# wvu-navLab/corenav-GP

Measured on AMD Instinct MI355X. Metric: GP-fits/s, higher is better.
Workload: dtype f64; 1 GPU; BASELINE configs[1]: batch of independent fixed-theta GP fits, N=2048 d=6 M=599 kernel=SE-ARD f64; streams=0, pipeline_depth=1, N=2048, d=6, M=599, inputs=resident in HBM, ranks=1

## Files before the change

### corenav_gp_amd/csrc/cgp_kernels_fused.hpp

```cpp
#pragma once
#include "cgp_kernels.hpp"

namespace cgp {

#ifndef CGP_SKIP_DEAD_WAVE
#define CGP_SKIP_DEAD_WAVE 1
#endif
constexpr bool kSkipDeadWave = CGP_SKIP_DEAD_WAVE != 0;

template <typename T>
__device__ __forceinline__ void stage_first_chunk(const T *gR, size_t ldR, const T *gC, size_t ldC, T *smem, int tid) {
  constexpr int CH = KT * LDST;
  if constexpr (sizeof(T) == 8) {
    typedef __attribute__((address_space(3))) void lds_void;
    typedef const __attribute__((address_space(1))) void gbl_void;
    const int lane = tid & 63;
    const int wave = __builtin_amdgcn_readfirstlane(tid >> 6);
#pragma unroll
    for (int i = 0; i < KT / 4; ++i) {
      const int col = wave * (KT / 4) + i;
      __builtin_amdgcn_global_load_lds((gbl_void *)(gR + (size_t)col * ldR + lane * 2), (lds_void *)(smem + col * LDST), 16, 0, 0);
      __builtin_amdgcn_global_load_lds((gbl_void *)(gC + (size_t)col * ldC + lane * 2), (lds_void *)(smem + CH + col * LDST), 16, 0, 0);
    }
  } else {
// ... 731 lines not shown
  const bf8 c01[2] = {__builtin_bit_cast(bf8, a01[RB0]), __builtin_bit_cast(bf8, a01[RB1])};
  static_for<0, RB1 + 1>([&](auto cc) {
    constexpr int CB = decltype(cc)::value;
    const bf8 a = __builtin_bit_cast(bf8, a01[CB]);
    if constexpr (CB <= RB0) acc[CB][0] = __builtin_amdgcn_mfma_f32_16x16x32_bf16(a, c10[0], acc[CB][0], 0, 0, 0);
    acc[CB][1] = __builtin_amdgcn_mfma_f32_16x16x32_bf16(a, c10[1], acc[CB][1], 0, 0, 0);
  });
  static_for<0, RB1 + 1>([&](auto cc) {
    constexpr int CB = decltype(cc)::value;
    const bf8 a = __builtin_bit_cast(bf8, a01[CB]);
    if constexpr (CB <= RB0) acc[CB][0] = __builtin_amdgcn_mfma_f32_16x16x32_bf16(a, c01[0], acc[CB][0], 0, 0, 0);
    acc[CB][1] = __builtin_amdgcn_mfma_f32_16x16x32_bf16(a, c01[1], acc[CB][1], 0, 0, 0);
  });
}
template <int D, int W, int S>
__device__ __forceinline__ void bx6_tri_iter(Prec<float>::acc_t (&acc)[NCB][2], BxTriStage<D> &st, int c, int nchunk, float *smem, const unsigned (&e)[2], bool hi) {
  st.template load<S>(c + D);
  lds_barrier();
  bx6_tri_compute<W, (S & 1) * 6 * BX_PLANE>(acc, e, hi);
  if (c + 1 < nchunk) st.template store<(S + 1) % D>(smem + ((S + 1) & 1) * BXT_FLOATS);
}
template <int D, int W>
__device__ __forceinline__ void bx6_tri_wave(Prec<float>::acc_t (&acc)[NCB][2], BxTriStage<D> &st, int nchunk, float *smem, int tid) {
  const int lane = tid & 63, l15 = lane & 15, lq = lane >> 4;
  const unsigned base = (unsigned)(size_t)smem;
  const unsigned e[2] = {base + 2 * bx_pos(l15, lq & 1), base + 2 * (bx_pos(DB + l15, lq & 1) - DB * BXS)};
  st.template store<0>(smem);
  for (int c0 = 0; c0 < nchunk; c0 += D) {
    bx6_tri_iter<D, W, 0>(acc, st, c0, nchunk, smem, e, lq >> 1);
    bx6_tri_iter<D, W, 1>(acc, st, c0 + 1, nchunk, smem, e, lq >> 1);
    if (D > 2) bx6_tri_iter<D, W, 2 % D>(acc, st, c0 + 2, nchunk, smem, e, lq >> 1);
    if (D > 2) bx6_tri_iter<D, W, 3 % D>(acc, st, c0 + 3, nchunk, smem, e, lq >> 1);
  }
}
template <int D>
__device__ __forceinline__ void bx6_syrk_tri_loop(Prec<float>::acc_t (&acc)[NCB][2], BxTriStage<D> &st, int nchunk, float *smem, int tid) {
  if (nchunk <= 0) return;
  const int wave = __builtin_amdgcn_readfirstlane(tid >> 6);
  switch (wave) {
    case 0: bx6_tri_wave<D, 0>(acc, st, nchunk, smem, tid); break;
    case 1: bx6_tri_wave<D, 1>(acc, st, nchunk, smem, tid); break;
    case 2: bx6_tri_wave<D, 2>(acc, st, nchunk, smem, tid); break;
    default: bx6_tri_wave<D, 3>(acc, st, nchunk, smem, tid); break;
  }
}

__device__ __forceinline__ double exp_gen(double x, const ExpC &e) { return exp_nonpos(x, e); }
__device__ __forceinline__ float exp_gen(float x, const ExpC &) { return __expf(fmaxf(x, -104.f)); }

constexpr int GK = 12;
template <bool DBL> constexpr int bx_z_offset() { return DBL ? 2 * BX_FLOATS : BX_FLOATS + 2 * GK * TS + 3 * TS; }
static_assert(2 * GK * TS + 3 * TS <= BX_FLOATS, "Gram inputs fit the second plane buffer");

template <typename T, bool BROWN, bool FAST, bool TRI = false, int NR = 2, bool DIFF1 = false, int MAT = 0>
__device__ __forceinline__ void gram_apply_tile(const FitArgs &p, typename Prec<T>::acc_t (&acc)[NCB][NR],
                                                const T *__restrict__ xrT, const T *__restrict__ xcT,
                                                const T *__restrict__ xraw, const T *__restrict__ craw,
                                                const T *__restrict__ yc, bool extra, int rowbase, int colbase, T amp,
                                                T amp_b, T diag_add, int lane, int wave, T inv_ell = T(0)) {
  using P = Prec<T>;
  using acc_t = typename P::acc_t;
  const int N = p.N, M = p.M, l15 = lane & 15, lq = lane >> 4;
  ExpC ec;
  ec.load();
  static_assert(NR == 2 || (NR == 1 && !TRI), "row blocks per wave");
  const int rbj[2] = {TRI ? wave : 0, TRI ? NCB - 1 - wave : 0};
  const int rl[2] = {TRI ? rbj[0] * DB + l15 : (NR == 2 ? wave * 32 + 2 * l15 : wave * DB + l15),
                     TRI ? rbj[1] * DB + l15 : wave * 32 + 2 * l15 + 1};
  T fb[NR][GK / 4];
#pragma unroll
  for (int j = 0; j < NR; ++j)
#pragma unroll
    for (int s = 0; s < GK / 4; ++s) fb[j][s] = xrT[(4 * s + lq) * TS + rl[j]];
  static_assert(!DIFF1 || (!BROWN && sizeof(T) == 4), "the difference form is for the fp32 SE kernels");
  static_assert(MAT == 0 || (!BROWN && !DIFF1 && sizeof(T) == 8), "the Matern kernels are fp64 cases of the inner-product form");
  T xrw[2] = {T(0), T(0)};
  if (BROWN || DIFF1) {
    xrw[0] = xraw[rl[0]];
    if (NR == 2) xrw[1] = xraw[rl[1]];
  }
#pragma unroll
  for (int cb = 0; cb < NCB; ++cb) {
    if (TRI && cb > rbj[0] && cb > rbj[1]) continue;
    T fa[GK / 4];
#pragma unroll
    for (int s = 0; s < GK / 4; ++s) fa[s] = xcT[(4 * s + lq) * TS + cb * DB + l15];
#pragma unroll
    for (int j = 0; j < NR; ++j) {
      if (TRI && cb > rbj[j]) continue;
      acc_t e = acc_t{0, 0, 0, 0};
      if constexpr (!DIFF1) {
#pragma unroll
        for (int s = 0; s < GK / 4; ++s) e = P::mfma(fa[s], fb[j][s], e);
      }
      const int grow = rowbase + rl[j];
#pragma unroll
      for (int r = 0; r < 4; ++r) {
        const int cl = cb * DB + P::drow(lane, r);
        const int gcol = colbase + cl;
        T g;
        if constexpr (DIFF1) {
          const T df = (xrw[j] - craw[cl]) * inv_ell;
          g = amp * exp_gen(T(-0.5) * df * df, ec);
        } else if constexpr (MAT != 0) {
          const bool same = !FAST && !extra && grow == gcol;
          double unused;
          g = amp * T(matern_radial<MAT == 2, false>(same ? 0.0 : -2.0 * (double)e[r], unused, [&](double x) { return exp_nonpos(x, ec); }));
        } else if (!BROWN) {
          g = CGP_DBG_ON(p, 128) ? e[r] : exp_gen(e[r], ec);
        } else {
          const T x = xrw[j], xp = craw[cl];
          const bool same = !FAST && !extra && grow == gcol;
          T ee = e[r] > T(0) ? T(0) : e[r];
          if constexpr (sizeof(T) == 4) {
            const T df = (x - xp) * inv_ell;
            ee = T(-0.5) * df * df;
          }
          ee = same ? T(0) : ee;
          const int sx = (x > T(0)) - (x < T(0)), sp = (xp > T(0)) - (xp < T(0));
          const T ax = x < T(0) ? -x : x, ap = xp < T(0) ? -xp : xp;
          const T kb = (sx == sp) ? amp_b * (ax < ap ? ax : ap) : T(0);
          g = amp * exp_gen(ee, ec) * kb;
        }
        if (!FAST) {
          const bool colok = gcol < N;
          if (!extra) {
            const bool dg = grow == gcol;
            g = dg ? g + diag_add : g;
            g = (grow < N && colok) ? g : (dg ? T(1) : T(0));
          } else {
            if (p.xid) g = (grow == gcol) ? T(1) : T(0);
            g = (grow == M) ? yc[cl] : g;
            g = (!colok || grow > M) ? T(0) : g;
          }
        }
        acc[cb][j][r] = -g;
      }
    }
    __builtin_amdgcn_sched_barrier(0);
  }
}

__global__ void k_prep(FitArgs p, int batch, double *prep, int zero_info, int *wready) {
  const int b = blockIdx.x * blockDim.x + threadIdx.x;
  if (b >= batch) return;
  if (zero_info) p.info[b] = 0;
  if (wready) wready[b] = 0;
  const double *th = p.theta + (size_t)b * MAX_THETA;
  double *o = prep + (size_t)b * PREP_N;
  const int kid = p.kernel_id, d = p.d;
  for (int q = 0; q < MAXD; ++q) {
    double s = 0.0;
    if (q < d) s = k_is_ard(kid) ? 1.0 / th[1 + q] : 1.0 / th[1];
    o[q] = s;
  }
  const bool brown = kid == K_RBF_BROWNIAN;
  o[8] = (brown || k_is_matern(kid)) ? 0.0 : log(th[0]);
  o[9] = th[0];
  o[10] = brown ? th[2] : 0.0;
  const int nth = k_ntheta(kid, d);
  o[11] = th[nth - 1] + 1e-8 + (p.jitter ? p.jitter[b] : 0.0);
  for (int q = 12; q < PREP_N; ++q) o[q] = 0.0;
}

template <typename T> struct GramPre {
  T v[MAXD];
  T yv;
};

template <typename T>
__device__ __forceinline__ void gram_prefetch(const FitArgs &p, int b, int k, int rt, int tid, GramPre<T> &g, int row0 = -1) {
  const int d = p.d, N = p.N, M = p.M;
  const bool extra = rt >= p.NT;
  const T *__restrict__ Xb = reinterpret_cast<const T *>(p.X) + (size_t)b * d * N;
  const T *__restrict__ Xsb = reinterpret_cast<const T *>(p.Xs) + (size_t)b * d * M;
  const T *__restrict__ yb = reinterpret_cast<const T *>(p.y) + (size_t)b * N;
  const bool isrow = tid < TS;
  const int r = tid & 127;
  const T *src = Xb;
  int idx, len = N;
  if (isrow) {
    if (!extra) idx = (row0 >= 0 ? row0 : rt * TS) + r;
    else { src = Xsb; idx = (row0 >= 0 ? row0 : (rt - p.NT) * TS) + r; len = M; }
  } else idx = k * TS + r;
  const bool ok = idx < len;
#pragma unroll
  for (int q = 0; q < MAXD; ++q) g.v[q] = (q < d && ok) ? src[(size_t)q * len + idx] : T(0);
  g.yv = (!isrow && ok) ? yb[idx] : T(0);
}

template <typename T, bool TRI = false, int NR = 2, bool MAT = false>
__device__ __forceinline__ void gram_apply(const FitArgs &p, typename Prec<T>::acc_t (&acc)[NCB][NR], T *__restrict__ smem,
                                           int b, int k, int rt, int tid, const GramPre<T> &g, PhaseClock *pc = nullptr,
                                           int slot = 0, int row0 = -1, bool live = true) {
  const double *__restrict__ pr = p.prep + (size_t)b * PREP_N;
  const int kid = p.kernel_id, N = p.N, M = p.M;
  const bool extra = rt >= p.NT;
  const bool brown = kid == K_RBF_BROWNIAN;
  const int lane = tid & 63;
  const int wave = __builtin_amdgcn_readfirstlane(tid >> 6);
  T *xrT = smem;
  T *xcT = smem + GK * TS;
  T *xraw = smem + 2 * GK * TS;
  T *craw = xraw + TS;
  T *yc = craw + TS;
  {
    const bool isrow = tid < TS;
    const int r = tid & 127;
    T *dst = isrow ? xrT : xcT;
    T nrm = 0;
#pragma unroll
    for (int q = 0; q < MAXD; ++q) {
      const T v = g.v[q] * T(pr[q]);
      nrm = __builtin_fma(v, v, nrm);
      dst[q * TS + r] = v;
    }
    dst[MAXD * TS + r] = isrow ? (T(-0.5) * nrm + T(pr[8])) : T(1);
    dst[(MAXD + 1) * TS + r] = isrow ? T(1) : T(-0.5) * nrm;
    dst[(MAXD + 2) * TS + r] = T(0);
    dst[(MAXD + 3) * TS + r] = T(0);
    if (isrow) xraw[r] = g.v[0];
    else {
      craw[r] = g.v[0];
      yc[r] = g.yv;
    }
  }
  __syncthreads();
  if (pc) pc->lap(p, slot);
  const T amp = T(pr[9]), amp_b = T(pr[10]), diag_add = T(pr[11]);
  const int rowbase = row0 >= 0 ? row0 : (extra ? (rt - p.NT) * TS : rt * TS);
  const int colbase = k * TS;
  constexpr int ROWS = NR == 2 ? TS : TS / 2;
  const bool fast = (colbase + TS <= N) && (extra ? (rowbase + ROWS <= M && !p.xid) : (rt != k && rowbase + ROWS <= N));
  if (!live) return;
  if constexpr (sizeof(T) == 4) {
    if (!brown && p.d == 1) {
      if constexpr (TRI) gram_apply_tile<T, false, false, true, NR, true>(p, acc, xrT, xcT, xraw, craw, yc, extra, rowbase, colbase, amp, amp_b, diag_add, lane, wave, T(pr[0]));
      else if (fast) gram_apply_tile<T, false, true, false, NR, true>(p, acc, xrT, xcT, xraw, craw, yc, extra, rowbase, colbase, amp, amp_b, diag_add, lane, wave, T(pr[0]));
      else gram_apply_tile<T, false, false, false, NR, true>(p, acc, xrT, xcT, xraw, craw, yc, extra, rowbase, colbase, amp, amp_b, diag_add, lane, wave, T(pr[0]));
      return;
    }
  }
  static_assert(!MAT || sizeof(T) == 8, "the Matern kernels are fp64 only");
  if constexpr (MAT) {
#define CGP_MATERN_TILE(FAST_, TRI_)                                                                                                  \
  do {                                                                                                                                \
    if (kid == K_MATERN52_ARD)                                                                                                        \
      gram_apply_tile<T, false, FAST_, TRI_, NR, false, 2>(p, acc, xrT, xcT, xraw, craw, yc, extra, rowbase, colbase, amp, amp_b, diag_add, lane, wave); \
    else                                                                                                                              \
      gram_apply_tile<T, false, FAST_, TRI_, NR, false, 1>(p, acc, xrT, xcT, xraw, craw, yc, extra, rowbase, colbase, amp, amp_b, diag_add, lane, wave); \
  } while (0)
    if constexpr (TRI) CGP_MATERN_TILE(false, true);
    else if (fast) CGP_MATERN_TILE(true, false);
    else CGP_MATERN_TILE(false, false);
#undef CGP_MATERN_TILE
    return;
  }
  if constexpr (TRI) {
    if (brown) gram_apply_tile<T, true, false, true>(p, acc, xrT, xcT, xraw, craw, yc, extra, rowbase, colbase, amp, amp_b, diag_add, lane, wave, T(pr[0]));
    else gram_apply_tile<T, false, false, true>(p, acc, xrT, xcT, xraw, craw, yc, extra, rowbase, colbase, amp, amp_b, diag_add, lane, wave);
  } else if (brown) {
    if (fast) gram_apply_tile<T, true, true, false, NR>(p, acc, xrT, xcT, xraw, craw, yc, extra, rowbase, colbase, amp, amp_b, diag_add, lane, wave, T(pr[0]));
    else gram_apply_tile<T, true, false, false, NR>(p, acc, xrT, xcT, xraw, craw, yc, extra, rowbase, colbase, amp, amp_b, diag_add, lane, wave, T(pr[0]));
  } else {
    if (fast) gram_apply_tile<T, false, true, false, NR>(p, acc, xrT, xcT, xraw, craw, yc, extra, rowbase, colbase, amp, amp_b, diag_add, lane, wave);
    else gram_apply_tile<T, false, false, false, NR>(p, acc, xrT, xcT, xraw, craw, yc, extra, rowbase, colbase, amp, amp_b, diag_add, lane, wave);
  }
}

__device__ __forceinline__ constexpr int tri_blk(int i, int j) { return (i * (i + 1) / 2 + j) * DB * DB; }
template <typename T> constexpr int diag_lds_elems() { return 36 * DB * DB + 3 * DB * DB; }

template <typename T>
__device__ __forceinline__ void diag_factor_packed(const FitArgs &p, T *__restrict__ Bk, T *__restrict__ tile, int ld,
                                                   T *__restrict__ Wk, int b, int k, int tid) {
  using P = Prec<T>;
  using acc_t = typename P::acc_t;
  constexpr int NB = TS / DB;
  const int lane = tid & 63;
  const int wave = __builtin_amdgcn_readfirstlane(tid >> 6);
  const int l15 = lane & 15, lq = lane >> 4;
  const int live = p.N - k * TS;
  T *Dv = Bk + 36 * DB * DB;
  T *DvT = Dv + DB * DB;
  int bad = 0;
  for (int jb = 0; jb < NB; ++jb) {
    const int j0 = jb * DB;
    if (wave == 0) {
      T *Djj = Bk + tri_blk(jb, jb);
      T a[DB], w[DB];
      if (j0 < live) {
#pragma unroll
        for (int c = 0; c < DB; ++c) a[c] = Djj[c * DB + l15];
        factor_block16<T>(a, w, bad, k * TS + j0, l15, [&] {
#pragma unroll
          for (int c = 0; c < DB; ++c) a[c] = Djj[c * DB + l15];
        });
      } else {
#pragma unroll
        for (int c = 0; c < DB; ++c) a[c] = w[c] = (c == l15) ? T(1) : T(0);
      }
      if (lane < DB) {
        T *dvt = DvT + (jb & 1) * DB * DB;
#pragma unroll
        for (int i = 0; i < DB; ++i) {
          Dv[l15 * DB + i] = w[i];
          dvt[i * DB + l15] = w[i];
          Wk[wimg_blk(jb, jb) + l15 * DB + i] = -w[i];
        }
#pragma unroll
        for (int c = 0; c < DB; ++c) tile[(size_t)(j0 + c) * ld + j0 + l15] = (l15 >= c) ? a[c] : T(0);
      }
    } else if (jb > 0) {
      const int pj = jb - 1;
      const T *dvt = DvT + (pj & 1) * DB * DB;
      for (int i = jb + wave - 1; i < NB; i += 3) {
        T *blk = Bk + tri_blk(i, pj);
        T fa[4], fb[4];
#pragma unroll
// ... 173 lines not shown
    potf2_tile<T>(p, At, Dv, Ts, flag, tile, ld, b, kn, tid);
    if (pc) {
      pc->lap(p, 347);
      pc->count(p, 351);
    }
    return;
  }
  if constexpr (TRI) {
#pragma unroll
    for (int cb = 0; cb < NCB; ++cb)
#pragma unroll
      for (int j = 0; j < 2; ++j) {
        const int rb = j ? NCB - 1 - wave : wave;
        if (cb <= rb) {
#pragma unroll
          for (int r = 0; r < 4; ++r) smem[tri_blk(rb, cb) + P::drow(lane, r) * DB + l15] = -acc[cb][j][r];
        }
      }
  } else {
    const int rb = 2 * wave + (l15 >> 3), rin = (2 * l15) & 15;
#pragma unroll
    for (int cb = 0; cb < NCB; ++cb)
      if (cb <= rb) {
#pragma unroll
        for (int r = 0; r < 4; ++r) {
          vec2 v;
          v[0] = -acc[cb][0][r];
          v[1] = -acc[cb][1][r];
          *reinterpret_cast<vec2 *>(smem + tri_blk(rb, cb) + P::drow(lane, r) * DB + rin) = v;
        }
      }
  }
  __syncthreads();
  T *Wk = reinterpret_cast<T *>(p.Winv) + (size_t)b * p.winv_stride + (size_t)kn * WIMG;
  if (pc) pc->lap(p, 346);
  diag_factor_packed<T>(p, smem, tile, ld, Wk, b, kn, tid);
  if (pc) {
    pc->lap(p, 347);
    pc->count(p, 351);
  }
}

template <typename T, bool FAT = false, bool MAT = false>
__global__ __launch_bounds__(256, 2) void k_diag_lean(FitArgs p, int k) {
  extern __shared__ __attribute__((aligned(16))) char smem_raw[];
  T *smem = reinterpret_cast<T *>(smem_raw);
  const int b = blockIdx.x;
  T *Lw = reinterpret_cast<T *>(p.Lw) + (size_t)b * p.lw_stride;
  typename Prec<T>::acc_t acc[NCB][2];
  diag_next<T, DIAG_FULL, kTriDiag, sizeof(T) == 8 || FAT, FAT, MAT>(p, acc, smem, Lw, b, k, threadIdx.x);
}

template <typename T>
__device__ __forceinline__ void trmm_in_registers(const FitArgs &p, typename Prec<T>::acc_t (&acc)[NCB][2], T *__restrict__ smem,
                                                  int b, int k, int tid, PhaseClock *pc = nullptr, int wslot = 0, bool live = true) {
  using P = Prec<T>;
  using acc_t = typename P::acc_t;
  const int lane = tid & 63, l15 = lane & 15;
  const T *__restrict__ Wk = reinterpret_cast<const T *>(p.Winv) + (size_t)b * p.winv_stride + (size_t)k * WIMG;
  {
    typedef __attribute__((address_space(3))) void lds_void;
    typedef const __attribute__((address_space(1))) void gbl_void;
    const int wave = __builtin_amdgcn_readfirstlane(tid >> 6);
    constexpr int PER = 1024 / (int)sizeof(T);
    constexpr int NI = WIMG / PER / 4;
    static_assert(WIMG % (4 * PER) == 0, "image is a whole number of 4 KiB rounds");
#pragma unroll
    for (int i = 0; i < NI; ++i) {
      const int off = (i * 4 + wave) * PER;
      __builtin_amdgcn_global_load_lds((gbl_void *)(Wk + off + lane * (16 / (int)sizeof(T))), (lds_void *)(smem + off), 16, 0, 0);
    }
    asm volatile("s_waitcnt vmcnt(0)" ::: "memory");
  }
  __syncthreads();
  if (pc) pc->lap(p, wslot);
  if (!live) return;

#pragma unroll
  for (int cb = NCB - 1; cb >= 0; --cb) {
    acc_t t0 = acc_t{0, 0, 0, 0}, t1 = t0;
    const T *wrow = smem + (cb * (cb + 1) / 2) * DB * DB + l15;
#pragma unroll
    for (int qb = 0; qb <= cb; ++qb) {
#pragma unroll
      for (int r = 0; r < 4; ++r) {
        const T a = wrow[qb * DB * DB + P::drow(lane, r) * DB];
        t0 = P::mfma(a, acc[qb][0][r], t0);
        t1 = P::mfma(a, acc[qb][1][r], t1);
      }
    }
    acc[cb][0] = t0;
    acc[cb][1] = t1;
    __builtin_amdgcn_sched_barrier(0);
  }
}

__device__ __forceinline__ void trmm_bx6_operand(int round, int ci, int &m, int &cb) {
  if (round) { m = 0; cb = ci; }
  else if (ci < 2) { m = 3; cb = 6 + ci; }
  else if (ci < 6) { m = 2; cb = 2 + ci; }
  else { m = 1; cb = ci - 4; }
}
template <int M, int CI0>
__device__ __forceinline__ void trmm_bx6_pair(Prec<float>::acc_t (&acc)[NCB][2], const unsigned short *planes, int lane) {
  using acc_t = Prec<float>::acc_t;
  bf8 bp[2][3];
#pragma unroll
  for (int j = 0; j < 2; ++j) {
    const float v[8] = {acc[2 * M][j][0], acc[2 * M][j][1], acc[2 * M][j][2], acc[2 * M][j][3],
                        acc[2 * M + 1][j][0], acc[2 * M + 1][j][1], acc[2 * M + 1][j][2], acc[2 * M + 1][j][3]};
    bxu4 w[3];
    bx_split8(v, w);
#pragma unroll
    for (int pl = 0; pl < 3; ++pl) bp[j][pl] = __builtin_bit_cast(bf8, w[pl]);
    acc[2 * M][j] = acc_t{0, 0, 0, 0};
    acc[2 * M + 1][j] = acc_t{0, 0, 0, 0};
  }
  static_for<0, (NCB - 2 * M) / 2>([&](auto hc) {
    constexpr int H = decltype(hc)::value, CB = 2 * M + 2 * H, CI = CI0 + 2 * H;
    bf8 ap[2][3];
#pragma unroll
    for (int u = 0; u < 2; ++u)
#pragma unroll
      for (int pl = 0; pl < 3; ++pl) ap[u][pl] = bx_ld8(planes + (((CI + u) * 3 + pl) * 64 + lane) * 8);
    constexpr int NT8 = 8;
    constexpr int TA[NT8] = {1, 2, 0, 2, 1, 0, 1, 0}, TB[NT8] = {2, 1, 2, 0, 1, 1, 0, 0};
// ... 188 lines not shown
    else if constexpr (BX6) bx6_loop<BXD, BXDBL>(acc, bxs, nchunk, smem, tid, accm ? zs : nullptr, ms, live);
    else mfma_rowpanel_loop<T, true>(acc, gR, (size_t)ld, gC, (size_t)ld, nchunk, smem, tid, accm ? zs : nullptr, ms, live);
  }
  pc.lap(p, ps + 1);
  if (accm) {
#pragma unroll
    for (int q = 0; q < 4; ++q) {
      ms[q] += __shfl_xor(ms[q], 16);
      ms[q] += __shfl_xor(ms[q], 32);
    }
    const int lane = tid & 63;
    const int wave = __builtin_amdgcn_readfirstlane(tid >> 6);
    if (lane < 16) {
#pragma unroll
      for (int j = 0; j < 2; ++j) {
        const int m = (rt - p.NT) * TS + wave * 32 + 2 * lane + j;
        if (m < p.M) {
          double *pm = p.macc + (size_t)b * p.M + m, *pv = p.vacc + (size_t)b * p.M + m;
          const double om = k == 1 ? 0.0 : __hip_atomic_load(pm, __ATOMIC_RELAXED, __HIP_MEMORY_SCOPE_AGENT);
          const double ov = k == 1 ? 0.0 : __hip_atomic_load(pv, __ATOMIC_RELAXED, __HIP_MEMORY_SCOPE_AGENT);
          __hip_atomic_store(pm, om + (double)ms[j], __ATOMIC_RELAXED, __HIP_MEMORY_SCOPE_AGENT);
          __hip_atomic_store(pv, ov + (double)ms[2 + j], __ATOMIC_RELAXED, __HIP_MEMORY_SCOPE_AGENT);
        }
      }
    }
  }
  __syncthreads();
  pc.lap(p, ps + 2);
  if (!CGP_DBG_ON(p, 64)) {
    if constexpr (kF32Bf16x6 && kBxTrmm && sizeof(T) == 4) trmm_bx6(p, acc, smem, b, k, tid, &pc, ps + 3, live);
    else trmm_in_registers<T>(p, acc, smem, b, k, tid, &pc, ps + 3, live);
  }
  pc.lap(p, ps + 4);
  if (live && (!CGP_DBG_ON(p, 32768) || acc[0][0][0] == T(12345.678)))
  store_tile<T>(acc, Lw + (size_t)(k * TS) * ld + (size_t)rt * TS, ld, tid);
  if constexpr (PL) {
    if (live) store_tile_planes(acc, reinterpret_cast<unsigned short *>(p.Lp) + (size_t)b * p.lp_stride, p.lp_stride / 3, ld, rt, k, tid);
  }
  pc.lap(p, ps + 5);
  pc.count(p, ps + 7);
  if constexpr (DIAGNEXT) {
    if (finish_next) {
      bool img_ready = false;
      if constexpr (MID && CGP_IMG_EARLY) {
        if (k + 1 >= 3) {
          const T *img = reinterpret_cast<const T *>(p.dpart) + ((size_t)b * img_slots(p) + (k + 1) % img_slots(p)) * DPART;
          acc_image<T, kTriDiag, false>(acc, const_cast<T *>(img), tid);
          img_ready = true;
        }
      }
      diag_next<T, DIAG_FINISH, kTriDiag, DEEP, mid_fat<T, MID>(), MAT>(p, acc, smem, Lw, b, k + 1, tid, &pc, img_ready);
    }
  }
}

#ifndef CGP_KINDA_PRIO
#define CGP_KINDA_PRIO 0
#endif
#ifndef CGP_F32_FULL_OCC
#define CGP_F32_FULL_OCC 4
#endif
constexpr int F32_FULL_OCC = CGP_F32_FULL_OCC;
template <typename T, bool DIAGNEXT = false, bool DEEP = sizeof(T) == 8, bool MID = false, bool MAT = false>
__global__ __launch_bounds__(256, sizeof(T) == 4 ? (DEEP ? ((MID && (CGP_MID_RING > 4 || CGP_F32_BF16X6)) ? 2 : 3) : F32_FULL_OCC) : 2) void k_panel(FitArgs p, int k) {
  using P = Prec<T>;
  using acc_t = typename P::acc_t;
  extern __shared__ __attribute__((aligned(16))) char smem_raw[];
  T *smem = reinterpret_cast<T *>(smem_raw);
  const int tid = threadIdx.x;
  int bt, b, rt;
  int c_first = 0;
  bool finish_next = false, from_image = false;
  acc_t acc[NCB][2];
  SpanClock sc;
  sc.enter(p, k, tid);
  if constexpr (DIAGNEXT) {
    const int Tg = gridDim.x, B = gridDim.y;
    const int lin = blockIdx.y * Tg + blockIdx.x;
    const int nA = (p.diag_slots & 1) ? B : 0, nB = (p.diag_slots & 2) ? B : 0, nC = (MID && (p.diag_slots & 4)) ? B : 0;
    int ia = -1, io = lin;
    const int stride = p.diag_stride, ablk = nA >> 8, oblk = (Tg * B - nA) >> 8;
    if (nA > 0 && (B & 255) == 0 && stride > 0 && (ablk - 1) * stride < ablk + oblk) {
      const int j = lin >> 8, r = lin & 255;
      const int before = min((j + stride - 1) / stride, ablk);
      if (j % stride == 0 && j / stride < ablk) ia = (j / stride) * 256 + r;
      else io = (j - before) * 256 + r;
    } else if (lin < nA) ia = lin;
    else io = lin - nA;
    if (CGP_DBG_ON(p, 65536) && (ia >= 0 || io < nB)) {
      if (ia < 0) return;
    }
    if (ia >= 0) {
      b = ia;
      rt = k + 1;
      finish_next = !CGP_DBG_ON(p, 65536);
      if constexpr (MID && CGP_KINDA_PRIO > 0) __builtin_amdgcn_s_setprio(CGP_KINDA_PRIO);
      if (MID && (p.diag_slots & 8)) {
        from_image = true;
        c_first = (k - 1) * (TS / KT);
      }
    } else if (io < nB) {
      b = io;
      T *LwB = reinterpret_cast<T *>(p.Lw) + (size_t)b * p.lw_stride;
      diag_next<T, DIAG_PARTIAL, kTriDiag, DEEP, false, MAT>(p, acc, smem, LwB, b, k + 2, tid);
      sc.leave(p, k, tid);
      return;
    } else if (MID && io < nB + nC) {
      panel_partial<T, DEEP, MAT>(p, acc, smem, io - nB, k, tid);
      sc.leave(p, k, tid);
      return;
    } else {
      const int l2 = io - nB - nC, To = Tg - (nA ? 1 : 0) - (nB ? 1 : 0) - (nC ? 1 : 0);
      if ((B & 7) == 0) {
        const int xcd = l2 & 7, slot = l2 >> 3;
        bt = slot % To;
        b = (slot / To) * 8 + xcd;
      } else {
        bt = l2 % To;
        b = l2 / To;
      }
      const int first = k + 1 + (nA ? 1 : 0);
      const int nin = p.NT - first > 0 ? p.NT - first : 0;
      rt = bt < nin ? first + bt : p.NT + (bt - nin);
    }
  } else {
    tile_fit_of_block(bt, b);
    rt = row_tile_of(bt + p.tile_off, k + 1, p.NT, p.rows_from_extra);
  }
  panel_tile_body<T, DIAGNEXT, DEEP, MID, MAT>(p, k, b, rt, c_first, finish_next, from_image, smem, tid);
  sc.leave(p, k, tid);
}

constexpr int HR = TS / 2;
template <typename T, int SLOT>
__device__ __forceinline__ void r16_load(T (&f)[4][KT / 4], const T *gRl, size_t ldR, int chunk, int lq) {
#pragma unroll
  for (int ks = 0; ks < KT / 4; ++ks) {
    const T *src = gRl + (size_t)(chunk * KT + ks * 4 + lq) * ldR;
    if constexpr (sizeof(T) == 8) asm volatile("global_load_dwordx2 %0, %1, off" : "=&v"(f[SLOT][ks]) : "v"(src));
    else asm volatile("global_load_dword %0, %1, off" : "=&v"(f[SLOT][ks]) : "v"(src));
  }
}
template <typename T, int S, bool ISSUE, int WAITN, bool ACC>
__device__ __forceinline__ void r16_step(typename Prec<T>::acc_t (&acc)[NCB][1], T (&f)[4][KT / 4], const T *gRl, size_t ldR, const T *gC,
                                         size_t ldC, int c, T *smem, int lane, int wave, const T *zs, T *ms) {
  using P = Prec<T>;
  constexpr int CH = KT * LDST;
  const int l15 = lane & 15, lq = lane >> 4;
  asm volatile("s_waitcnt vmcnt(%0)\n\ts_barrier" ::"n"(WAITN) : "memory");
#pragma unroll
  for (int ks = 0; ks < KT / 4; ++ks) asm volatile("" : "+v"(f[S][ks]));
  if constexpr (ISSUE) {
    cpanel_stage<T>(gC, ldC, c + 2, smem + ((S + 2) & 3) * CH, lane, wave);
    r16_load<T, (S + 2) & 3>(f, gRl, ldR, c + 2, lq);
  }
  const T *cur = smem + S * CH + lq * LDST + l15;
  T fa[2][NCB];
#pragma unroll
  for (int cb = 0; cb < NCB; ++cb) fa[0][cb] = cur[cb * DB];
#pragma unroll
  for (int ks = 0; ks < KT / 4; ++ks) {
    if (ks + 1 < KT / 4) {
#pragma unroll
      for (int cb = 0; cb < NCB; ++cb) fa[(ks + 1) & 1][cb] = cur[(ks + 1) * 4 * LDST + cb * DB];
    }
    const T fb = f[S][ks];
    if constexpr (ACC) {
      const T zv = zs[ks * 4 + lq];
      ms[0] = __builtin_fma(fb, zv, ms[0]);
      ms[1] = __builtin_fma(fb, fb, ms[1]);
    }
#pragma unroll
    for (int cb = 0; cb < NCB; ++cb) acc[cb][0] = P::mfma(fa[ks & 1][cb], fb, acc[cb][0]);
  }
}

template <typename T, bool MAT = false>
__global__ __launch_bounds__(256, sizeof(T) == 4 ? 4 : 2) void k_rows64(FitArgs p, int k) {
  using P = Prec<T>;
  using acc_t = typename P::acc_t;
// ... 699 lines not shown
```

Before: 11270 fits/s.

## Add 2x2 wave-split panel path for partially filled last extra row tile

Adds a specialized fp64 panel tile body for the last extra (test-point) row tile when it holds only a few 16-row blocks. Waves are split 2x2 over row and column halves, so only the live row blocks are loaded, multiplied and stored, and the TRMM hands the lower column half's accumulators across waves through LDS. It also reorders the block-to-tile mapping so blocks running the short last tile are dealt after the long ones. This avoids padded MFMA work on the ragged M=599 tail, at the cost of extra LDS exchange, barriers and code size.

```diff
diff --git a/corenav_gp_amd/csrc/cgp_kernels_fused.hpp b/corenav_gp_amd/csrc/cgp_kernels_fused.hpp
--- a/corenav_gp_amd/csrc/cgp_kernels_fused.hpp
+++ b/corenav_gp_amd/csrc/cgp_kernels_fused.hpp
@@ -807,8 +807,8 @@
 template <bool DBL> constexpr int bx_z_offset() { return DBL ? 2 * BX_FLOATS : BX_FLOATS + 2 * GK * TS + 3 * TS; }
 static_assert(2 * GK * TS + 3 * TS <= BX_FLOATS, "Gram inputs fit the second plane buffer");
 
-template <typename T, bool BROWN, bool FAST, bool TRI = false, int NR = 2, bool DIFF1 = false, int MAT = 0>
-__device__ __forceinline__ void gram_apply_tile(const FitArgs &p, typename Prec<T>::acc_t (&acc)[NCB][NR],
+template <typename T, bool BROWN, bool FAST, bool TRI = false, int NR = 2, bool DIFF1 = false, int MAT = 0, int NC = NCB>
+__device__ __forceinline__ void gram_apply_tile(const FitArgs &p, typename Prec<T>::acc_t (&acc)[NC][NR],
                                                 const T *__restrict__ xrT, const T *__restrict__ xcT,
                                                 const T *__restrict__ xraw, const T *__restrict__ craw,
                                                 const T *__restrict__ yc, bool extra, int rowbase, int colbase, T amp,
@@ -818,10 +818,17 @@
   const int N = p.N, M = p.M, l15 = lane & 15, lq = lane >> 4;
   ExpC ec;
   ec.load();
-  static_assert(NR == 2 || (NR == 1 && !TRI), "row blocks per wave");
+  static_assert(NC == NCB ? (NR == 2 || (NR == 1 && !TRI)) : (NC == 4 && NR >= 1 && NR <= 3 && !TRI && !DIFF1 && sizeof(T) == 8), "row blocks per wave");
+  constexpr int NRA = NR > 2 ? NR : 2;
   const int rbj[2] = {TRI ? wave : 0, TRI ? NCB - 1 - wave : 0};
-  const int rl[2] = {TRI ? rbj[0] * DB + l15 : (NR == 2 ? wave * 32 + 2 * l15 : wave * DB + l15),
-                     TRI ? rbj[1] * DB + l15 : wave * 32 + 2 * l15 + 1};
+  int rl[NRA];
+  rl[0] = TRI ? rbj[0] * DB + l15 : (NR == 2 ? wave * 32 + 2 * l15 : wave * DB + l15);
+  rl[1] = TRI ? rbj[1] * DB + l15 : wave * 32 + 2 * l15 + 1;
+  if constexpr (NC != NCB) {
+#pragma unroll
+    for (int j = 0; j < NR; ++j) rl[j] = ((wave >> 1) * NR + j) * DB + l15;
+  }
+  const int cb0 = NC == NCB ? 0 : (wave & 1) * NC;
   T fb[NR][GK / 4];
 #pragma unroll
   for (int j = 0; j < NR; ++j)
@@ -829,17 +836,19 @@
     for (int s = 0; s < GK / 4; ++s) fb[j][s] = xrT[(4 * s + lq) * TS + rl[j]];
   static_assert(!DIFF1 || (!BROWN && sizeof(T) == 4), "the difference form is for the fp32 SE kernels");
   static_assert(MAT == 0 || (!BROWN && !DIFF1 && sizeof(T) == 8), "the Matern kernels are fp64 cases of the inner-product form");
-  T xrw[2] = {T(0), T(0)};
+  T xrw[NRA];
+#pragma unroll
+  for (int j = 0; j < NRA; ++j) xrw[j] = T(0);
   if (BROWN || DIFF1) {
-    xrw[0] = xraw[rl[0]];
-    if (NR == 2) xrw[1] = xraw[rl[1]];
-  }
-#pragma unroll
-  for (int cb = 0; cb < NCB; ++cb) {
+#pragma unroll
+    for (int j = 0; j < NR; ++j) xrw[j] = xraw[rl[j]];
+  }
+#pragma unroll
+  for (int cb = 0; cb < NC; ++cb) {
     if (TRI && cb > rbj[0] && cb > rbj[1]) continue;
     T fa[GK / 4];
 #pragma unroll
-    for (int s = 0; s < GK / 4; ++s) fa[s] = xcT[(4 * s + lq) * TS + cb * DB + l15];
+    for (int s = 0; s < GK / 4; ++s) fa[s] = xcT[(4 * s + lq) * TS + (cb0 + cb) * DB + l15];
 #pragma unroll
     for (int j = 0; j < NR; ++j) {
       if (TRI && cb > rbj[j]) continue;
@@ -851,7 +860,7 @@
       const int grow = rowbase + rl[j];
 #pragma unroll
       for (int r = 0; r < 4; ++r) {
-        const int cl = cb * DB + P::drow(lane, r);
+        const int cl = (cb0 + cb) * DB + P::drow(lane, r);
         const int gcol = colbase + cl;
         T g;
         if constexpr (DIFF1) {
@@ -944,8 +953,8 @@
   g.yv = (!isrow && ok) ? yb[idx] : T(0);
 }
 
-template <typename T, bool TRI = false, int NR = 2, bool MAT = false>
-__device__ __forceinline__ void gram_apply(const FitArgs &p, typename Prec<T>::acc_t (&acc)[NCB][NR], T *__restrict__ smem,
+template <typename T, bool TRI = false, int NR = 2, bool MAT = false, int NC = NCB>
+__device__ __forceinline__ void gram_apply(const FitArgs &p, typename Prec<T>::acc_t (&acc)[NC][NR], T *__restrict__ smem,
                                            int b, int k, int rt, int tid, const GramPre<T> &g, PhaseClock *pc = nullptr,
                                            int slot = 0, int row0 = -1, bool live = true) {
   const double *__restrict__ pr = p.prep + (size_t)b * PREP_N;
@@ -985,8 +994,8 @@
   const T amp = T(pr[9]), amp_b = T(pr[10]), diag_add = T(pr[11]);
   const int rowbase = row0 >= 0 ? row0 : (extra ? (rt - p.NT) * TS : rt * TS);
   const int colbase = k * TS;
-  constexpr int ROWS = NR == 2 ? TS : TS / 2;
-  const bool fast = (colbase + TS <= N) && (extra ? (rowbase + ROWS <= M && !p.xid) : (rt != k && rowbase + ROWS <= N));
+  constexpr int ROWS = NC != NCB ? 2 * NR * DB : (NR == 2 ? TS : TS / 2);
+  const bool fast = NC == NCB && (colbase + TS <= N) && (extra ? (rowbase + ROWS <= M && !p.xid) : (rt != k && rowbase + ROWS <= N));
   if (!live) return;
   if constexpr (sizeof(T) == 4) {
     if (!brown && p.d == 1) {
@@ -1001,9 +1010,9 @@
 #define CGP_MATERN_TILE(FAST_, TRI_)                                                                                                  \
   do {                                                                                                                                \
     if (kid == K_MATERN52_ARD)                                                                                                        \
-      gram_apply_tile<T, false, FAST_, TRI_, NR, false, 2>(p, acc, xrT, xcT, xraw, craw, yc, extra, rowbase, colbase, amp, amp_b, diag_add, lane, wave); \
+      gram_apply_tile<T, false, FAST_, TRI_, NR, false, 2, NC>(p, acc, xrT, xcT, xraw, craw, yc, extra, rowbase, colbase, amp, amp_b, diag_add, lane, wave); \
     else                                                                                                                              \
-      gram_apply_tile<T, false, FAST_, TRI_, NR, false, 1>(p, acc, xrT, xcT, xraw, craw, yc, extra, rowbase, colbase, amp, amp_b, diag_add, lane, wave); \
+      gram_apply_tile<T, false, FAST_, TRI_, NR, false, 1, NC>(p, acc, xrT, xcT, xraw, craw, yc, extra, rowbase, colbase, amp, amp_b, diag_add, lane, wave); \
   } while (0)
     if constexpr (TRI) CGP_MATERN_TILE(false, true);
     else if (fast) CGP_MATERN_TILE(true, false);
@@ -1015,11 +1024,11 @@
     if (brown) gram_apply_tile<T, true, false, true>(p, acc, xrT, xcT, xraw, craw, yc, extra, rowbase, colbase, amp, amp_b, diag_add, lane, wave, T(pr[0]));
     else gram_apply_tile<T, false, false, true>(p, acc, xrT, xcT, xraw, craw, yc, extra, rowbase, colbase, amp, amp_b, diag_add, lane, wave);
   } else if (brown) {
-    if (fast) gram_apply_tile<T, true, true, false, NR>(p, acc, xrT, xcT, xraw, craw, yc, extra, rowbase, colbase, amp, amp_b, diag_add, lane, wave, T(pr[0]));
-    else gram_apply_tile<T, true, false, false, NR>(p, acc, xrT, xcT, xraw, craw, yc, extra, rowbase, colbase, amp, amp_b, diag_add, lane, wave, T(pr[0]));
+    if (fast) gram_apply_tile<T, true, true, false, NR, false, 0, NC>(p, acc, xrT, xcT, xraw, craw, yc, extra, rowbase, colbase, amp, amp_b, diag_add, lane, wave, T(pr[0]));
+    else gram_apply_tile<T, true, false, false, NR, false, 0, NC>(p, acc, xrT, xcT, xraw, craw, yc, extra, rowbase, colbase, amp, amp_b, diag_add, lane, wave, T(pr[0]));
   } else {
-    if (fast) gram_apply_tile<T, false, true, false, NR>(p, acc, xrT, xcT, xraw, craw, yc, extra, rowbase, colbase, amp, amp_b, diag_add, lane, wave);
-    else gram_apply_tile<T, false, false, false, NR>(p, acc, xrT, xcT, xraw, craw, yc, extra, rowbase, colbase, amp, amp_b, diag_add, lane, wave);
+    if (fast) gram_apply_tile<T, false, true, false, NR, false, 0, NC>(p, acc, xrT, xcT, xraw, craw, yc, extra, rowbase, colbase, amp, amp_b, diag_add, lane, wave);
+    else gram_apply_tile<T, false, false, false, NR, false, 0, NC>(p, acc, xrT, xcT, xraw, craw, yc, extra, rowbase, colbase, amp, amp_b, diag_add, lane, wave);
   }
 }
 
@@ -1299,26 +1308,30 @@
 }
 
 template <typename T>
+__device__ __forceinline__ void wk_stage(const FitArgs &p, T *__restrict__ smem, int b, int k, int tid) {
+  const int lane = tid & 63;
+  const T *__restrict__ Wk = reinterpret_cast<const T *>(p.Winv) + (size_t)b * p.winv_stride + (size_t)k * WIMG;
+  typedef __attribute__((address_space(3))) void lds_void;
+  typedef const __attribute__((address_space(1))) void gbl_void;
+  const int wave = __builtin_amdgcn_readfirstlane(tid >> 6);
+  constexpr int PER = 1024 / (int)sizeof(T);
+  constexpr int NI = WIMG / PER / 4;
+  static_assert(WIMG % (4 * PER) == 0, "image is a whole number of 4 KiB rounds");
+#pragma unroll
+  for (int i = 0; i < NI; ++i) {
+    const int off = (i * 4 + wave) * PER;
+    __builtin_amdgcn_global_load_lds((gbl_void *)(Wk + off + lane * (16 / (int)sizeof(T))), (lds_void *)(smem + off), 16, 0, 0);
+  }
+  asm volatile("s_waitcnt vmcnt(0)" ::: "memory");
+}
+
+template <typename T>
 __device__ __forceinline__ void trmm_in_registers(const FitArgs &p, typename Prec<T>::acc_t (&acc)[NCB][2], T *__restrict__ smem,
                                                   int b, int k, int tid, PhaseClock *pc = nullptr, int wslot = 0, bool live = true) {
   using P = Prec<T>;
   using acc_t = typename P::acc_t;
   const int lane = tid & 63, l15 = lane & 15;
-  const T *__restrict__ Wk = reinterpret_cast<const T *>(p.Winv) + (size_t)b * p.winv_stride + (size_t)k * WIMG;
-  {
-    typedef __attribute__((address_space(3))) void lds_void;
-    typedef const __attribute__((address_space(1))) void gbl_void;
-    const int wave = __builtin_amdgcn_readfirstlane(tid >> 6);
-    constexpr int PER = 1024 / (int)sizeof(T);
-    constexpr int NI = WIMG / PER / 4;
-    static_assert(WIMG % (4 * PER) == 0, "image is a whole number of 4 KiB rounds");
-#pragma unroll
-    for (int i = 0; i < NI; ++i) {
-      const int off = (i * 4 + wave) * PER;
-      __builtin_amdgcn_global_load_lds((gbl_void *)(Wk + off + lane * (16 / (int)sizeof(T))), (lds_void *)(smem + off), 16, 0, 0);
-    }
-    asm volatile("s_waitcnt vmcnt(0)" ::: "memory");
-  }
+  wk_stage<T>(p, smem, b, k, tid);
   __syncthreads();
   if (pc) pc->lap(p, wslot);
   if (!live) return;
@@ -1613,6 +1626,226 @@
       diag_next<T, DIAG_FINISH, kTriDiag, DEEP, mid_fat<T, MID>(), MAT>(p, acc, smem, Lw, b, k + 1, tid, &pc, img_ready);
     }
   }
+}
+
+#ifndef CGP_PANEL_2X2
+#define CGP_PANEL_2X2 1
+#endif
+constexpr bool kPanel2x2 = CGP_PANEL_2X2 != 0;
+constexpr int NC2 = NCB / 2;
+template <typename T, int RB> struct RowFrag2 {
+  T r[4][KT / 4][RB];
+};
+__device__ __forceinline__ int last_tile_rb(const FitArgs &p, int rt) {
+  if (rt != p.NT + p.ET - 1 || p.xid) return 0;
+  const int rows = p.M + 1 - (p.ET - 1) * TS;
+  return rows <= 6 * DB ? (rows + 2 * DB - 1) / (2 * DB) : 0;
+}
+
+template <typename T, int SLOT, int RB>
+__device__ __forceinline__ void rfrag2_load(RowFrag2<T, RB> &f, const T *gRl, size_t ldR, int chunk, int lq) {
+  static_assert(sizeof(T) == 8, "fp64 only");
+#pragma unroll
+  for (int ks = 0; ks < KT / 4; ++ks) {
+    const T *src = gRl + (size_t)(chunk * KT + ks * 4 + lq) * ldR;
+    asm volatile("global_load_dwordx2 %0, %1, off" : "=&v"(f.r[SLOT][ks][0]) : "v"(src));
+    if constexpr (RB > 1) asm volatile("global_load_dwordx2 %0, %1, off offset:%2" : "=&v"(f.r[SLOT][ks][1]) : "v"(src), "n"(DB * 8));
+    if constexpr (RB > 2) asm volatile("global_load_dwordx2 %0, %1, off offset:%2" : "=&v"(f.r[SLOT][ks][2]) : "v"(src), "n"(2 * DB * 8));
+    static_assert(RB <= 3, "row blocks per wave");
+  }
+}
+
+template <typename T, int RB, int S, bool ISSUE, int WAITN, bool ACC = false>
+__device__ __forceinline__ void rdirect2_step(typename Prec<T>::acc_t (&acc)[NC2][RB], RowFrag2<T, RB> &f, const T *gRl, size_t ldR,
+                                              const T *gC, size_t ldC, int c, T *smem, int lane, int wave, const T *zs = nullptr,
+                                              T *ms = nullptr) {
+  using P = Prec<T>;
+  constexpr int CH = KT * LDST;
+  const int l15 = lane & 15, lq = lane >> 4;
+  static_assert(WAITN >= 0 && WAITN <= 63, "vmcnt is a 6-bit counter");
+  asm volatile("s_waitcnt vmcnt(%0)\n\ts_barrier" ::"n"(WAITN) : "memory");
+#pragma unroll
+  for (int ks = 0; ks < KT / 4; ++ks)
+#pragma unroll
+    for (int rb = 0; rb < RB; ++rb) asm volatile("" : "+v"(f.r[S][ks][rb]));
+  if constexpr (ISSUE) {
+    cpanel_stage<T>(gC, ldC, c + 2, smem + ((S + 2) & 3) * CH, lane, wave);
+    rfrag2_load<T, (S + 2) & 3, RB>(f, gRl, ldR, c + 2, lq);
+  }
+  const T *cur = smem + S * CH + lq * LDST + (wave & 1) * (NC2 * DB) + l15;
+  T fa[2][NC2];
+#pragma unroll
+  for (int cb = 0; cb < NC2; ++cb) fa[0][cb] = cur[cb * DB];
+#pragma unroll
+  for (int ks = 0; ks < KT / 4; ++ks) {
+    if (ks + 1 < KT / 4) {
+#pragma unroll
+      for (int cb = 0; cb < NC2; ++cb) fa[(ks + 1) & 1][cb] = cur[(ks + 1) * 4 * LDST + cb * DB];
+    }
+    if constexpr (ACC) {
+      const T zv = zs[ks * 4 + lq];
+#pragma unroll
+      for (int rb = 0; rb < RB; ++rb) {
+        const T fb = f.r[S][ks][rb];
+        ms[rb] = __builtin_fma(fb, zv, ms[rb]);
+        ms[RB + rb] = __builtin_fma(fb, fb, ms[RB + rb]);
+      }
+    }
+#pragma unroll
+    for (int cb = 0; cb < NC2; ++cb)
+#pragma unroll
+      for (int rb = 0; rb < RB; ++rb) acc[cb][rb] = P::mfma(fa[ks & 1][cb], f.r[S][ks][rb], acc[cb][rb]);
+  }
+}
+
+template <typename T, int RB>
+__device__ __forceinline__ void rdirect2_prologue(RowFrag2<T, RB> &f, const T *gRl, size_t ldR, const T *gC, size_t ldC, int nchunk,
+                                                  T *smem, int lane, int wave) {
+  constexpr int CH = KT * LDST;
+  if (nchunk <= 0) return;
+  cpanel_stage<T>(gC, ldC, 0, smem, lane, wave);
+  rfrag2_load<T, 0, RB>(f, gRl, ldR, 0, lane >> 4);
+  cpanel_stage<T>(gC, ldC, 1, smem + CH, lane, wave);
+  rfrag2_load<T, 1, RB>(f, gRl, ldR, 1, lane >> 4);
+}
+
+template <typename T, int RB>
+__device__ __forceinline__ void mfma_rowpanel_loop_2x2(typename Prec<T>::acc_t (&acc)[NC2][RB], RowFrag2<T, RB> &f, const T *gRl,
+                                                       size_t ldR, const T *gC, size_t ldC, int nchunk, T *smem, int lane, int wave,
+                                                       const T *zs, T (&ms)[2 * RB]) {
+  if (nchunk <= 0) return;
+  constexpr int L = cpanel_loads<T>() + RB * (KT / 4);
+  static_assert(L <= 63, "vmcnt");
+  int c = 0;
+  for (; c + 8 < nchunk; c += 4) {
+    static_for<0, 4>([&](auto jc) {
+      constexpr int J = decltype(jc)::value;
+      rdirect2_step<T, RB, J, true, L>(acc, f, gRl, ldR, gC, ldC, c + J, smem, lane, wave);
+    });
+  }
+  static_for<0, 8>([&](auto jc) {
+    constexpr int J = decltype(jc)::value;
+    constexpr int behind = 1 < (7 - J) ? 1 : (7 - J);
+    rdirect2_step<T, RB, J & 3, (J + 2 < 8), behind * L, true>(acc, f, gRl, ldR, gC, ldC, c + J, smem, lane, wave, zs + J * KT, ms);
+  });
+}
+
+template <typename T, int RB>
+__device__ __forceinline__ void trmm_2x2(const FitArgs &p, typename Prec<T>::acc_t (&acc)[NC2][RB], T *__restrict__ smem, int b, int k,
+                                         int tid) {
+  using P = Prec<T>;
+  using acc_t = typename P::acc_t;
+  const int lane = tid & 63, l15 = lane & 15;
+  const int wave = __builtin_amdgcn_readfirstlane(tid >> 6);
+  const int wr = wave >> 1, wc = wave & 1;
+  static_assert(2 * RB * NC2 * 4 * 64 <= 4 * KT * LDST, "the hand-over fits the chunk ring");
+  acc_t lo[NC2][RB];
+  T *xch = smem + (size_t)wr * (RB * NC2 * 4 * 64) + lane;
+  if (wc == 0) {
+#pragma unroll
+    for (int cb = 0; cb < NC2; ++cb)
+#pragma unroll
+      for (int rb = 0; rb < RB; ++rb)
+#pragma unroll
+        for (int r = 0; r < 4; ++r) xch[((cb * RB + rb) * 4 + r) * 64] = acc[cb][rb][r];
+  }
+  __syncthreads();
+#pragma unroll
+  for (int cb = 0; cb < NC2; ++cb)
+#pragma unroll
+    for (int rb = 0; rb < RB; ++rb)
+#pragma unroll
+      for (int r = 0; r < 4; ++r) lo[cb][rb][r] = xch[((cb * RB + rb) * 4 + r) * 64];
+  __syncthreads();
+  wk_stage<T>(p, smem, b, k, tid);
+  __syncthreads();
+#pragma unroll
+  for (int cl = NC2 - 1; cl >= 0; --cl) {
+    const int cb = wc * NC2 + cl;
+    acc_t t[RB];
+#pragma unroll
+    for (int rb = 0; rb < RB; ++rb) t[rb] = acc_t{0, 0, 0, 0};
+    const T *wrow = smem + (cb * (cb + 1) / 2) * DB * DB + l15;
+    if (wc) {
+#pragma unroll
+      for (int qb = 0; qb < NC2; ++qb)
+#pragma unroll
+        for (int r = 0; r < 4; ++r) {
+          const T a = wrow[qb * DB * DB + P::drow(lane, r) * DB];
+#pragma unroll
+          for (int rb = 0; rb < RB; ++rb) t[rb] = P::mfma(a, lo[qb][rb][r], t[rb]);
+        }
+    }
+    const T *wown = wrow + wc * (NC2 * DB * DB);
+#pragma unroll
+    for (int j = 0; j <= cl; ++j)
+#pragma unroll
+      for (int r = 0; r < 4; ++r) {
+        const T a = wown[j * DB * DB + P::drow(lane, r) * DB];
+#pragma unroll
+        for (int rb = 0; rb < RB; ++rb) t[rb] = P::mfma(a, acc[j][rb][r], t[rb]);
+      }
+#pragma unroll
+    for (int rb = 0; rb < RB; ++rb) acc[cl][rb] = t[rb];
+    __builtin_amdgcn_sched_barrier(0);
+  }
+}
+
+template <typename T, int RB, bool MAT>
+__device__ __forceinline__ void panel_tile_body_2x2(const FitArgs &p, int k, int b, int rt, T *smem, int tid) {
+  using P = Prec<T>;
+  using acc_t = typename P::acc_t;
+  acc_t acc[NC2][RB];
+  T *Lw = reinterpret_cast<T *>(p.Lw) + (size_t)b * p.lw_stride;
+  const int ld = p.ld, lane = tid & 63, l15 = lane & 15;
+  const int wave = __builtin_amdgcn_readfirstlane(tid >> 6);
+  const int wr = wave >> 1, wc = wave & 1;
+  const T *gR = Lw + (size_t)rt * TS, *gC = Lw + (size_t)k * TS;
+  const T *gRl = gR + wr * (RB * DB) + l15;
+  const int nchunk = k * (TS / KT);
+  const bool accm = p.macc != nullptr && k > 0;
+  T *zs = smem + 4 * KT * LDST;
+  if (tid < TS) zs[tid] = accm ? Lw[(size_t)((k - 1) * TS + tid) * ld + (size_t)p.NT * TS + p.M] : T(0);
+  T ms[2 * RB];
+#pragma unroll
+  for (int q = 0; q < 2 * RB; ++q) ms[q] = T(0);
+  RowFrag2<T, RB> rf;
+  {
+    GramPre<T> gp;
+    gram_prefetch<T>(p, b, k, rt, tid, gp);
+    rdirect2_prologue<T, RB>(rf, gRl, (size_t)ld, gC, (size_t)ld, nchunk, smem, lane, wave);
+    gram_apply<T, false, RB, MAT, NC2>(p, acc, smem + 2 * KT * LDST, b, k, rt, tid, gp);
+  }
+  mfma_rowpanel_loop_2x2<T, RB>(acc, rf, gRl, (size_t)ld, gC, (size_t)ld, nchunk, smem, lane, wave, zs, ms);
+  if (accm) {
+#pragma unroll
+    for (int q = 0; q < 2 * RB; ++q) {
+      ms[q] += __shfl_xor(ms[q], 16);
+      ms[q] += __shfl_xor(ms[q], 32);
+    }
+    if (wc == 0 && lane < 16) {
+#pragma unroll
+      for (int rb = 0; rb < RB; ++rb) {
+        const int m = (rt - p.NT) * TS + (wr * RB + rb) * DB + lane;
+        if (m < p.M) {
+          double *pm = p.macc + (size_t)b * p.M + m, *pv = p.vacc + (size_t)b * p.M + m;
+          const double om = k == 1 ? 0.0 : __hip_atomic_load(pm, __ATOMIC_RELAXED, __HIP_MEMORY_SCOPE_AGENT);
+          const double ov = k == 1 ? 0.0 : __hip_atomic_load(pv, __ATOMIC_RELAXED, __HIP_MEMORY_SCOPE_AGENT);
+          __hip_atomic_store(pm, om + (double)ms[rb], __ATOMIC_RELAXED, __HIP_MEMORY_SCOPE_AGENT);
+          __hip_atomic_store(pv, ov + (double)ms[RB + rb], __ATOMIC_RELAXED, __HIP_MEMORY_SCOPE_AGENT);
+        }
+      }
+    }
+  }
+  __syncthreads();
+  trmm_2x2<T, RB>(p, acc, smem, b, k, tid);
+  T *__restrict__ out = Lw + (size_t)(k * TS) * ld + (size_t)rt * TS + wr * (RB * DB) + l15;
+#pragma unroll
+  for (int cb = 0; cb < NC2; ++cb)
+#pragma unroll
+    for (int r = 0; r < 4; ++r)
+#pragma unroll
+      for (int rb = 0; rb < RB; ++rb) out[(size_t)((wc * NC2 + cb) * DB + P::drow(lane, r)) * ld + rb * DB] = acc[cb][rb][r];
 }
 
 #ifndef CGP_KINDA_PRIO
@@ -1686,7 +1919,26 @@
     }
   } else {
     tile_fit_of_block(bt, b);
+    if constexpr (kPanel2x2 && sizeof(T) == 8 && DEEP && !MID && !MAT) {
+      constexpr int kDealLastFrom = 4;
+      const int Tg = gridDim.x, nb = gridDim.y >> 3;
+      if (k >= kDealLastFrom && (gridDim.y & 7) == 0 && Tg > 1 && !p.tile_off && last_tile_rb(p, p.NT + p.ET - 1)) {
+        const int lin = blockIdx.y * Tg + blockIdx.x, xcd = lin & 7, slot = lin >> 3, nlong = (Tg - 1) * nb;
+        bt = slot >= nlong ? Tg - 1 : slot % (Tg - 1);
+        b = (slot >= nlong ? slot - nlong : slot / (Tg - 1)) * 8 + xcd;
+      }
+    }
     rt = row_tile_of(bt + p.tile_off, k + 1, p.NT, p.rows_from_extra);
+    if constexpr (kPanel2x2 && sizeof(T) == 8 && DEEP && !MID && !MAT) {
+      const int rb2 = __builtin_amdgcn_readfirstlane(last_tile_rb(p, rt));
+      if (rb2) {
+        if (rb2 == 3) panel_tile_body_2x2<T, 3, MAT>(p, k, b, rt, smem, tid);
+        else if (rb2 == 2) panel_tile_body_2x2<T, 2, MAT>(p, k, b, rt, smem, tid);
+        else panel_tile_body_2x2<T, 1, MAT>(p, k, b, rt, smem, tid);
+        sc.leave(p, k, tid);
+        return;
+      }
+    }
   }
   panel_tile_body<T, DIAGNEXT, DEEP, MID, MAT>(p, k, b, rt, c_first, finish_next, from_image, smem, tid);
   sc.leave(p, k, tid);
```

Result: no change. 11380 fits/s, median of 6 (+1.0%).
